# shanice-l/UNOPose

Measured on AMD Instinct MI355X. Metric: (query,ref) pairs/sec forward, higher is better.
Workload: dtype bf16; 1 GPU; UNOPose.forward, batch 32 pairs/GPU, 2048 query pts, 5000->2048 reference pts, 196 coarse pts, 518x518 crops, DINOv2 ViT-B/14 reg4, random-init (trained-like) weights

## Files before the change

### unopose_amd/csrc/gemm_kernel.h

```cpp
#pragma once
#include "gemm_common.h"

namespace unopose {

constexpr int GEMM_XPOL = 2;
#define GEMM_BK 64
constexpr int GEMM_ROTX = 5, GEMM_ROTS = 3;

#define GEMM_WAIT_VM(n) asm volatile("s_waitcnt vmcnt(" #n ")" ::: "memory")
#define GEMM_WAIT_VM_(n) GEMM_WAIT_VM(n)

#define GEMM_LDS_BIAS (2 * GEMM_BUFBYTES)
#define GEMM_LDS_MBOX (GEMM_LDS_BIAS + 2048)
#define GEMM_LDS_LNW (GEMM_LDS_MBOX + 16)
#define GEMM_LDS_LNB (GEMM_LDS_LNW + 1024)
#define GEMM_LDS_LNPART (GEMM_LDS_LNB + 1024)
#define GEMM_LDS_STATS GEMM_LDS_LNPART
#define GEMM_LNF_MAXPARTS 4
#define GEMM_LDS_SHIFT (GEMM_LDS_LNPART + 8192)

template <int EPI, bool GATHER = false, bool F32 = false>
__global__ __launch_bounds__(512, 1) __attribute__((amdgpu_num_vgpr(127))) void gemm256_kernel(const void *__restrict__ Av, const void *__restrict__ Wv,
                                                           const float *__restrict__ bias, void *__restrict__ Cv, int M,
                                                           int N, int K, int tiles_n, int tiles_arg, int nt_store,
                                                           const int *__restrict__ row_list = nullptr,
                                                           const int *__restrict__ tile_info = nullptr,
                                                           const u16 *__restrict__ resid = nullptr, const float *__restrict__ ln_w = nullptr,
                                                           const float *__restrict__ ln_b = nullptr, float ln_eps = 0.f, int lda = 0,
                                                           int ldw = 0, int ldc = 0, int *__restrict__ sched = nullptr,
                                                           void *__restrict__ C2v = nullptr, const float *__restrict__ aux_vec = nullptr,
                                                           float2 *__restrict__ stats = nullptr, int nparts = 0, int stagger = 0,
                                                           const float *__restrict__ fold_prev = nullptr) {
  static_assert(!(F32 && (EPI == 3 || GATHER)), "the fp32-class form has no LayerNorm epilogue / gathered rows");
  static_assert(!((F32 || GATHER) && EPI >= 5), "the residual / LayerNorm-fold epilogues belong to the dense bf16 form");
  constexpr bool LNF = EPI == 6 || EPI == 7;
  static_assert(F32 || EPI != 4, "EPI 4 (bf16 + residual out of fp32-class operands) is an F32 epilogue");
  constexpr int ESZ = F32 ? 4 : 2;
  constexpr int KT = F32 ? 32 : 64;
  const char *A = reinterpret_cast<const char *>(Av), *W = reinterpret_cast<const char *>(Wv);
  const int LDA = lda ? lda : K, LDW = ldw ? ldw : K, LDC = ldc ? ldc : N;
  const int tiles = GATHER ? __builtin_amdgcn_readfirstlane(tile_info[0]) : tiles_arg;
  __shared__ __attribute__((aligned(1024))) char smem[GEMM_LDS_BIAS + 2048 + 16 + (EPI == 3 ? 2048 + 8192 : EPI == 5 ? 2048 + 8192 + 4096 : LNF ? 2048 + 2 * 8192 : 0)];
  float *const lnw_lds = reinterpret_cast<float *>(smem + GEMM_LDS_LNW), *const lnb_lds = reinterpret_cast<float *>(smem + GEMM_LDS_LNB);
  float2 *const ln_part = reinterpret_cast<float2 *>(smem + GEMM_LDS_LNPART);
  if (EPI == 3 && threadIdx.x < GEMM_BN) {
    lnw_lds[threadIdx.x] = ln_w[threadIdx.x];
    lnb_lds[threadIdx.x] = ln_b[threadIdx.x];
  }
  const int tid = threadIdx.x, lane = tid & 63, wave = __builtin_amdgcn_readfirstlane(tid >> 6);
  const int wm = wave >> 2, wn = wave & 3;
  const int l31 = lane & 31, hi = lane >> 5;
  const int l31_ = l31, hi_ = hi, lane_ = lane;
  const int xcd = blockIdx.x & 7, slot = blockIdx.x >> 3, nslots = gridDim.x >> 3;
  const int tiles_m = tiles / tiles_n, per_group = GEMM_GM * tiles_n;
  int cw = (size_t)N * K * ESZ > (size_t)(4u << 20) ? (2400 * 1024) / (GEMM_BN * K * ESZ) : 0;
  if (cw < 3) cw = 0;
  const bool colwalk = cw > 0 && !GATHER && tiles_n > cw && ((tiles_m & 7) == 0 || tiles_m >= 512);
  const int rq = tiles_m >> 3, rr = tiles_m & 7;
  const int rows_x = rq + (xcd < rr ? 1 : 0), row_base = xcd < rr ? xcd * (rq + 1) : rr * (rq + 1) + (xcd - rr) * rq;
  const int cq = tiles >> 3, cr = tiles & 7;
  const int chunk_base = xcd < cr ? xcd * (cq + 1) : cr * (cq + 1) + (xcd - cr) * cq;
  const int chunk_len = colwalk ? rows_x * tiles_n : cq + (xcd < cr ? 1 : 0);
  const __amdgpu_buffer_rsrc_t a_rs = __builtin_amdgcn_make_buffer_rsrc((void *)A, 0, (int)((size_t)M * LDA * ESZ), 0x00020000);
  const __amdgpu_buffer_rsrc_t w_rs = __builtin_amdgcn_make_buffer_rsrc((void *)W, 0, (int)((size_t)N * LDW * ESZ), 0x00020000);
  const __amdgpu_buffer_rsrc_t c_rs = __builtin_amdgcn_make_buffer_rsrc(Cv, 0, GATHER ? 0x7fffffff : (int)((size_t)M * LDC * 2), 0x00020000);
  const __amdgpu_buffer_rsrc_t b_rs = __builtin_amdgcn_make_buffer_rsrc((void *)bias, 0, N * 4, 0x00020000);
  const int nk = K / KT;

  const int fx = (l31 >> 1) & 7;
  uint32_t fr_off[4];
#pragma unroll
  for (int ks = 0; ks < 4; ++ks) fr_off[ks] = (uint32_t)((l31 >> 3) * 1024 + (l31 & 7) * 128 + ((((ks << 1) | hi) ^ fx) << 4));
  const uint32_t a_base = (uint32_t)(wm * 16384);
  const uint32_t w_base = (uint32_t)(GEMM_OPBYTES + wn * 8192);
  const uint32_t a_dst = (uint32_t)((wave >> 2) * 16384 + (wave & 3) * 2048);
  const uint32_t w_dst = (uint32_t)(GEMM_OPBYTES + (wave >> 1) * 8192 + (wave & 1) * 2048);

  struct TileP {
    int m0, n0, rot;
    uint32_t a_off[4], w_off[2];
  };
  auto tile_params = [&](int ti, int step, TileP &p) {
    const int t = chunk_base + ti;
    int tn, tm;
    if (GATHER) {
      tm = t;
      tn = 0;
      const int ng = N / GEMM_BN;
      for (int g = 1; g < ng; ++g) tn += t >= tile_info[1 + g] ? 1 : 0;
      tn = __builtin_amdgcn_readfirstlane(tn);
    } else if (colwalk) {
      const int per_block = rows_x * cw;
      const int cb = ti / per_block, v = ti - cb * per_block;
      const int cwb = min(cw, tiles_n - cb * cw);
      const int g = v / (GEMM_GM * cwb), w = v - g * GEMM_GM * cwb;
      const int gm = min(GEMM_GM, rows_x - g * GEMM_GM);
      const int tl = w / gm;
      tn = cb * cw + tl;
      tm = row_base + g * GEMM_GM + (w - tl * gm);
    } else {
      const int mg = t / per_group, rr = t - mg * per_group;
      const int gm = min(GEMM_GM, tiles_m - mg * GEMM_GM);
      tn = rr / gm;
      tm = mg * GEMM_GM + (rr - tn * gm);
    }
// ... 70 lines not shown
    __syncthreads();
    ti = __builtin_amdgcn_readfirstlane(mbox[0]);
  }
  if (EPI == 5 && stagger > 0 && ((slot / tiles_n) & 1)) {
    const uint64_t t0 = __builtin_amdgcn_s_memrealtime();
    while ((int64_t)(__builtin_amdgcn_s_memrealtime() - t0) < (int64_t)stagger) __builtin_amdgcn_s_sleep(8);
  }
  for (; ti < chunk_len;) {
    const int step = dyn ? ti / nslots : (ti - slot) / nslots;
    if (!have) {
      tile_params(ti, step, cur);
      stage_bias(cur, bsel);
      stage_half(cur, H_A0, 0, par);
      stage_half(cur, H_B0, 0, par);
      stage_half(cur, H_B1, 0, par);
      stage_half(cur, H_A1, 0, par);
      if (nk >= 2) {
        stage_half(cur, H_A0, 1, par ^ GEMM_BUFBYTES);
        stage_half(cur, H_B0, 1, par ^ GEMM_BUFBYTES);
        GEMM_WAIT_VM(6);
      } else {
        GEMM_WAIT_VM(2);
      }
      asm volatile("s_waitcnt lgkmcnt(0)" ::: "memory");
      __builtin_amdgcn_s_barrier();
    }
    const int m0 = __builtin_amdgcn_readfirstlane(cur.m0), n0 = __builtin_amdgcn_readfirstlane(cur.n0);
    cur.rot = __builtin_amdgcn_readfirstlane(cur.rot);
    bool more = can_stream && ti + nslots < chunk_len;
    int ti_next = ti + nslots;
    TileP nxt;

    const float *bias_lds = reinterpret_cast<const float *>(smem + GEMM_LDS_BIAS + bsel * 1024);
    f32x16 acc[2][4];
#pragma unroll
    for (int nb = 0; nb < 2; ++nb)
#pragma unroll
      for (int g = 0; g < 4; ++g) {
        const float4 bv = EPI == 3 || LNF ? make_float4(0.f, 0.f, 0.f, 0.f) : *reinterpret_cast<const float4 *>(bias_lds + wn * 64 + nb * 32 + 8 * g + 4 * hi);
#pragma unroll
        for (int mb = 0; mb < 4; ++mb) {
          acc[nb][mb][4 * g + 0] = bv.x;
          acc[nb][mb][4 * g + 1] = bv.y;
          acc[nb][mb][4 * g + 2] = bv.z;
          acc[nb][mb][4 * g + 3] = bv.w;
        }
      }

    bf16x8 af[2][4], wf0[4], wf1[4];
    auto read_a = [&](const char *lb, int ah) {
#pragma unroll
      for (int mbl = 0; mbl < 2; ++mbl)
#pragma unroll
        for (int ks = 0; ks < 4; ++ks) af[mbl][ks] = *reinterpret_cast<const bf16x8 *>(lb + a_base + ah * 8192 + mbl * 4096 + fr_off[ks]);
    };
    auto read_b = [&](const char *lb, int bh, bf16x8(&wf)[4]) {
#pragma unroll
      for (int ks = 0; ks < 4; ++ks) wf[ks] = *reinterpret_cast<const bf16x8 *>(lb + w_base + bh * 4096 + fr_off[ks]);
    };
    auto mfma_q = [&](int ah, int bh, const bf16x8(&wf)[4]) {
      if (F32) {
#pragma unroll
        for (int b = 0; b < 2; ++b)
#pragma unroll
          for (int mbl = 0; mbl < 2; ++mbl) {
            f32x16 &a = acc[bh][2 * ah + mbl];
            a = __builtin_amdgcn_mfma_f32_32x32x16_bf16(wf[2 + b], af[mbl][b], a, 0, 0, 0);
            a = __builtin_amdgcn_mfma_f32_32x32x16_bf16(wf[b], af[mbl][2 + b], a, 0, 0, 0);
            a = __builtin_amdgcn_mfma_f32_32x32x16_bf16(wf[b], af[mbl][b], a, 0, 0, 0);
          }
        return;
      }
#pragma unroll
      for (int ks = 0; ks < 4; ++ks)
#pragma unroll
        for (int mbl = 0; mbl < 2; ++mbl)
          acc[bh][2 * ah + mbl] = __builtin_amdgcn_mfma_f32_32x32x16_bf16(wf[ks], af[mbl][ks], acc[bh][2 * ah + mbl], 0, 0, 0);
    };
    if (wm == 1) __builtin_amdgcn_s_barrier();
    auto phase = [&](auto compute) {
      asm volatile("s_waitcnt lgkmcnt(0)" ::: "memory");
      __builtin_amdgcn_sched_barrier(0);
      __builtin_amdgcn_s_barrier();
      __builtin_amdgcn_sched_barrier(0);
      compute();
      __builtin_amdgcn_sched_barrier(0);
      __builtin_amdgcn_s_barrier();
      asm volatile("" ::: "memory");
      __builtin_amdgcn_sched_barrier(0);
    };
    for (int t = 0; t < nk; ++t) {
      const bool last = t + 1 == nk, last2 = t + 2 >= nk;
      if (dyn) {
        if (t == 2 && wave == 0) {
          int tk;
          asm volatile("v_readfirstlane_b32 %0, v255" : "=s"(tk)::"memory");
          if (lane == 0) mbox[0] = tk;
        }
        if (t + 2 == nk) {
          ti_next = __builtin_amdgcn_readfirstlane(*reinterpret_cast<volatile int *>(mbox));
          more = ti_next < chunk_len;
        }
      }
      if (more && t + 2 == nk) tile_params(ti_next, dyn ? ti_next / nslots : step + 1, nxt);
      const char *lb = smem + par;
      const uint32_t bnext = par ^ GEMM_BUFBYTES;
      read_b(lb, 0, wf0);
      read_b(lb, 1, wf1);
      read_a(lb, 0);
      __builtin_amdgcn_sched_barrier(0);
// ... 28 lines not shown
        stage_half(cur, H_B0, t + 2, par);
        stage_half(cur, H_B1, t + 2, par);
        GEMM_WAIT_VM(8);
      } else if (more) {
        if (!last) {
          stage_bias(nxt, bsel ^ 1);
          stage_half(nxt, H_A0, 0, par);
          stage_half(nxt, H_B0, 0, par);
          stage_half(nxt, H_B1, 0, par);
          if (LNF) {
            if (nparts <= 3) GEMM_WAIT_VM(9);
            else GEMM_WAIT_VM(10);
          } else
            GEMM_WAIT_VM(8);
        } else if (F32) {
          GEMM_WAIT_VM(2);
        } else {
          stage_half(nxt, H_A0, 1, par);
          stage_half(nxt, H_B0, 1, par);
          GEMM_WAIT_VM(6);
        }
      } else if (!last) {
        GEMM_WAIT_VM(2);
      }
      phase([&] {
        mfma_q(1, 1, wf1);
        mfma_q(1, 0, wf0);
      });
      par ^= GEMM_BUFBYTES;
    }
    if (wm == 0) __builtin_amdgcn_s_barrier();
    par ^= GEMM_BUFBYTES;
    if (EPI == 3) {
#pragma unroll
      for (int mb = 0; mb < 4; ++mb) {
        const int m = min(m0 + wm * 128 + mb * 32 + l31, M - 1);
        const u16 *rp = resid + (size_t)m * GEMM_BN + wn * 64 + 4 * hi;
        float a1 = 0.f, a2 = 0.f;
#pragma unroll
        for (int nb = 0; nb < 2; ++nb)
#pragma unroll
          for (int g = 0; g < 4; ++g) {
            const int nl = nb * 32 + 8 * g + 4 * hi;
            const float4 bv = *reinterpret_cast<const float4 *>(bias_lds + wn * 64 + nl);
            const uint2 r = *reinterpret_cast<const uint2 *>(rp + nb * 32 + 8 * g);
            const float v0 = acc[nb][mb][4 * g + 0] + bv.x + __uint_as_float(r.x << 16);
            const float v1 = acc[nb][mb][4 * g + 1] + bv.y + __uint_as_float(r.x & 0xffff0000u);
            const float v2 = acc[nb][mb][4 * g + 2] + bv.z + __uint_as_float(r.y << 16);
            const float v3 = acc[nb][mb][4 * g + 3] + bv.w + __uint_as_float(r.y & 0xffff0000u);
            acc[nb][mb][4 * g + 0] = v0;
            acc[nb][mb][4 * g + 1] = v1;
            acc[nb][mb][4 * g + 2] = v2;
            acc[nb][mb][4 * g + 3] = v3;
            a1 += (v0 + v1) + (v2 + v3);
            a2 += (v0 * v0 + v1 * v1) + (v2 * v2 + v3 * v3);
          }
        a1 += __shfl_xor(a1, 32);
        a2 += __shfl_xor(a2, 32);
        if (hi == 0) ln_part[((wm * 4 + mb) * 32 + l31) * 4 + wn] = make_float2(a1, a2);
      }
      __syncthreads();
#pragma unroll
      for (int mb = 0; mb < 4; ++mb) {
        const float2 *pp = ln_part + ((wm * 4 + mb) * 32 + l31) * 4;
        const float t1 = (pp[0].x + pp[1].x) + (pp[2].x + pp[3].x), t2 = (pp[0].y + pp[1].y) + (pp[2].y + pp[3].y);
        const float mean = t1 * (1.f / GEMM_BN);
        const float rstd = rsqrtf(fmaxf(t2 * (1.f / GEMM_BN) - mean * mean, 0.f) + ln_eps);
#pragma unroll
        for (int nb = 0; nb < 2; ++nb)
#pragma unroll
          for (int g = 0; g < 4; ++g) {
            const int nl = wn * 64 + nb * 32 + 8 * g + 4 * hi;
            const float4 gw = *reinterpret_cast<const float4 *>(lnw_lds + nl), gb = *reinterpret_cast<const float4 *>(lnb_lds + nl);
            acc[nb][mb][4 * g + 0] = (acc[nb][mb][4 * g + 0] - mean) * rstd * gw.x + gb.x;
            acc[nb][mb][4 * g + 1] = (acc[nb][mb][4 * g + 1] - mean) * rstd * gw.y + gb.y;
            acc[nb][mb][4 * g + 2] = (acc[nb][mb][4 * g + 2] - mean) * rstd * gw.z + gb.z;
            acc[nb][mb][4 * g + 3] = (acc[nb][mb][4 * g + 3] - mean) * rstd * gw.w + gb.w;
          }
      }
    }
    if constexpr (LNF) {
      int l31 = l31_, hi = hi_;
      asm volatile("" : "+v"(l31), "+v"(hi));
      const float *c_lds = reinterpret_cast<const float *>(smem + GEMM_LDS_LNW + bsel * 1024);
      const float inv_k = 1.f / (float)K;
      float rs[4], nm[4];
#pragma unroll
      for (int mb = 0; mb < 4; ++mb) {
        const float2 *sp = reinterpret_cast<const float2 *>(smem + GEMM_LDS_STATS + bsel * 8192) + (wm * 128 + mb * 32 + l31) * nparts;
        float t1 = 0.f, t2 = 0.f;
#pragma unroll
        for (int i = 0; i < GEMM_LNF_MAXPARTS; ++i)
          if (i < nparts) {
            const float2 q = sp[i];
            t1 += q.x;
            t2 += q.y;
          }
        const float mean = t1 * inv_k;
        rs[mb] = rsqrtf(fmaxf(t2 * inv_k - mean * mean, 0.f) + ln_eps);
        nm[mb] = -mean * rs[mb];
      }
#pragma unroll
      for (int nb = 0; nb < 2; ++nb)
#pragma unroll
        for (int g = 0; g < 4; ++g) {
          const int nl = wn * 64 + nb * 32 + 8 * g + 4 * hi;
          const float4 cv = *reinterpret_cast<const float4 *>(c_lds + nl), dv = *reinterpret_cast<const float4 *>(bias_lds + nl);
#pragma unroll
          for (int mb = 0; mb < 4; ++mb) {
            acc[nb][mb][4 * g + 0] = fmaf(rs[mb], acc[nb][mb][4 * g + 0], fmaf(nm[mb], cv.x, dv.x));
            acc[nb][mb][4 * g + 1] = fmaf(rs[mb], acc[nb][mb][4 * g + 1], fmaf(nm[mb], cv.y, dv.y));
            acc[nb][mb][4 * g + 2] = fmaf(rs[mb], acc[nb][mb][4 * g + 2], fmaf(nm[mb], cv.z, dv.z));
            acc[nb][mb][4 * g + 3] = fmaf(rs[mb], acc[nb][mb][4 * g + 3], fmaf(nm[mb], cv.w, dv.w));
          }
        }
    }
    if constexpr (EPI == 5) {
      int l31 = l31_, hi = hi_, lane = lane_;
      asm volatile("" : "+v"(l31), "+v"(hi), "+v"(lane));
      char *cw = smem + par + (wave < 4 ? 8192 + (wave & 1) * 4096 + (wave >> 1) * 16384 : GEMM_OPBYTES + 4096 + (wave - 4) * 8192);
      const __amdgpu_buffer_rsrc_t x_rs = __builtin_amdgcn_make_buffer_rsrc(C2v, 0, (int)((size_t)M * N * 4), 0x00020000);
      const int r4 = lane >> 4, q = lane & 15;
      const uint32_t x_v0 = (uint32_t)((((size_t)m0 + wm * 128 + r4) * N + n0 + wn * 64 + q * 4) * 4);
      const uint32_t c_v0 = (uint32_t)((((size_t)m0 + wm * 128 + r4) * LDC + n0 + wn * 64 + q * 4) * 2);
      const uint32_t x_rowb = (uint32_t)(N * 4), c_rowb = (uint32_t)(LDC * 2);
      const int rows_p = tiles_m * GEMM_BM;
      float sv[2] = {0.f, 0.f};
      if (fold_prev != nullptr) {
        float pv[2][GEMM_LNF_MAXPARTS + 1];
#pragma unroll
        for (int j = 0; j < 2; ++j) {
          const size_t m = (size_t)m0 + wm * 128 + j * 64 + lane, sh_at = (size_t)rows_p * 2 * nparts + m;
#pragma unroll
          for (int i = 0; i < GEMM_LNF_MAXPARTS; ++i) pv[j][i] = fold_prev[i < nparts ? m * 2 * nparts + 2 * i : sh_at];
          pv[j][GEMM_LNF_MAXPARTS] = fold_prev[sh_at];
        }
#pragma unroll
        for (int j = 0; j < 2; ++j) {
          float t = 0.f;
#pragma unroll
          for (int i = 0; i < GEMM_LNF_MAXPARTS; ++i) t += i < nparts ? pv[j][i] : 0.f;
          sv[j] = m0 + wm * 128 + j * 64 + lane < M ? pv[j][GEMM_LNF_MAXPARTS] + t * (1.f / (float)N) : 0.f;
        }
      }
      constexpr int PF = 3;
      f32x4 rv[PF][4];
      auto load_round = [&](int r, f32x4(&dst)[4]) {
#pragma unroll
        for (int it = 0; it < 4; ++it) {
          dst[it] = __builtin_bit_cast(f32x4, __builtin_amdgcn_raw_buffer_load_b128(x_rs, x_v0 + (uint32_t)(r * 16 + it * 4) * x_rowb, 0, GEMM_XPOL));
        }
      };
#pragma unroll
      for (int r = 0; r < PF; ++r) load_round(r, rv[r]);
      float *const sh_lds = reinterpret_cast<float *>(smem + GEMM_LDS_SHIFT + wave * 512);
#pragma unroll
      for (int r = 0; r < 8; ++r) {
        const int mb = r >> 1, h = r & 1;
        if ((l31 >> 4) == h) {
#pragma unroll
          for (int nb = 0; nb < 2; ++nb)
#pragma unroll
            for (int g = 0; g < 4; ++g) {
              const int s16 = (nb * 8 + 2 * g + hi) ^ (l31 & 15);
              *reinterpret_cast<float4 *>(cw + (l31 & 15) * 256 + s16 * 16) =
                  make_float4(acc[nb][mb][4 * g + 0], acc[nb][mb][4 * g + 1], acc[nb][mb][4 * g + 2], acc[nb][mb][4 * g + 3]);
            }
        }
        if (r == 0) {
#pragma unroll
          for (int j = 0; j < 2; ++j) {
            sh_lds[j * 64 + lane] = sv[j];
            if (wn == 0) reinterpret_cast<float *>(stats)[(size_t)rows_p * 2 * tiles_n + m0 + wm * 128 + j * 64 + lane] = sv[j];
          }
        }
        __builtin_amdgcn_fence(__ATOMIC_RELEASE, "wavefront");
        __builtin_amdgcn_wave_barrier();
        __builtin_amdgcn_fence(__ATOMIC_ACQUIRE, "wavefront");
#pragma unroll
        for (int it = 0; it < 4; ++it) {
          const int row = it * 4 + r4;
          const f32x4 a = *reinterpret_cast<const f32x4 *>(cw + row * 256 + ((q ^ row) << 4));
          const f32x4 o = rv[r % PF][it];
          f32x4 v;
#pragma unroll
          for (int e = 0; e < 4; ++e) v[e] = a[e] + o[e];
          __builtin_amdgcn_raw_buffer_store_b128(__builtin_bit_cast(u32x4, v), x_rs, x_v0 + (uint32_t)(r * 16 + it * 4) * x_rowb, 0, GEMM_XPOL);
          const float s = sh_lds[row + r * 16];
#pragma unroll
          for (int e = 0; e < 4; ++e) v[e] = v[e] - s;
          typedef unsigned int u32x2 __attribute__((ext_vector_type(2)));
          const u32x2 pk = {cvt_pk_bf16_f32(v[0], v[1]), cvt_pk_bf16_f32(v[2], v[3])};
          if (nt_store)
            __builtin_amdgcn_raw_buffer_store_b64(pk, c_rs, c_v0 + (uint32_t)(r * 16 + it * 4) * c_rowb, 0, 2);
          else
            __builtin_amdgcn_raw_buffer_store_b64(pk, c_rs, c_v0 + (uint32_t)(r * 16 + it * 4) * c_rowb, 0, 0);
          float a1 = (v[0] + v[1]) + (v[2] + v[3]), a2 = (v[0] * v[0] + v[1] * v[1]) + (v[2] * v[2] + v[3] * v[3]);
          a1 += dpp_f32<0x111, 0xF>(a1, 0.f);
          a2 += dpp_f32<0x111, 0xF>(a2, 0.f);
          a1 += dpp_f32<0x112, 0xF>(a1, 0.f);
          a2 += dpp_f32<0x112, 0xF>(a2, 0.f);
          a1 += dpp_f32<0x114, 0xF>(a1, 0.f);
          a2 += dpp_f32<0x114, 0xF>(a2, 0.f);
          a1 += dpp_f32<0x118, 0xF>(a1, 0.f);
          a2 += dpp_f32<0x118, 0xF>(a2, 0.f);
          if (q == 15) ln_part[((wm * 4 + mb) * 32 + h * 16 + row) * 4 + wn] = make_float2(a1, a2);
        }
        __builtin_amdgcn_fence(__ATOMIC_RELEASE, "wavefront");
        __builtin_amdgcn_wave_barrier();
        __builtin_amdgcn_fence(__ATOMIC_ACQUIRE, "wavefront");
        if (r + PF < 8) load_round(r + PF, rv[r % PF]);
      }
      asm volatile("s_waitcnt lgkmcnt(0)" ::: "memory");
      __builtin_amdgcn_s_barrier();
      if (wn == 0 && hi == 0) {
#pragma unroll
        for (int mb = 0; mb < 4; ++mb) {
          const float2 *pp = ln_part + ((wm * 4 + mb) * 32 + l31) * 4;
          const float4 p01 = *reinterpret_cast<const float4 *>(pp), p23 = *reinterpret_cast<const float4 *>(pp + 2);
          stats[(size_t)(m0 + wm * 128 + mb * 32 + l31) * tiles_n + (n0 >> 8)] = make_float2((p01.x + p01.z) + (p23.x + p23.z), (p01.y + p01.w) + (p23.y + p23.w));
        }
      }
    } else if constexpr (!F32) {
    int l31 = l31_, hi = hi_, lane = lane_;
    asm volatile("" : "+v"(l31), "+v"(hi), "+v"(lane));
    char *cw = smem + par + (wave < 4 ? 8192 + (wave & 1) * 4096 + (wave >> 1) * 16384 : GEMM_OPBYTES + 4096 + (wave - 4) * 8192);
    const uint32_t c_v0 = GATHER ? (uint32_t)((((size_t)m0 + wm * 128 + (lane >> 3)) * GEMM_BN + wn * 64 + (lane & 7) * 8) * 2)
                                 : (uint32_t)((((size_t)m0 + wm * 128 + (lane >> 3)) * LDC + n0 + wn * 64 + (lane & 7) * 8) * 2);
    const uint32_t c_rowb = (uint32_t)((GATHER ? GEMM_BN : LDC) * 2);
#pragma unroll
    for (int mb = 0; mb < 4; ++mb) {
#pragma unroll
      for (int nb = 0; nb < 2; ++nb) {
#pragma unroll
        for (int g = 0; g < 4; ++g) {
          const int nl = nb * 32 + 8 * g + 4 * hi;
          float v0 = acc[nb][mb][4 * g + 0], v1 = acc[nb][mb][4 * g + 1], v2 = acc[nb][mb][4 * g + 2], v3 = acc[nb][mb][4 * g + 3];
          if (EPI == 1 || EPI == 7) {
            v0 = gelu_bf16_class(v0);
            v1 = gelu_bf16_class(v1);
            v2 = gelu_bf16_class(v2);
            v3 = gelu_bf16_class(v3);
          }
          if (EPI == 2) {
            v0 = fmaxf(v0, 0.f);
            v1 = fmaxf(v1, 0.f);
            v2 = fmaxf(v2, 0.f);
            v3 = fmaxf(v3, 0.f);
          }
          const int slot16 = (nl >> 3) ^ (l31 & 7);
          *reinterpret_cast<uint2 *>(cw + l31 * 128 + slot16 * 16 + (nl & 4) * 2) = make_uint2(cvt_pk_bf16_f32(v0, v1), cvt_pk_bf16_f32(v2, v3));
        }
      }
      __builtin_amdgcn_fence(__ATOMIC_RELEASE, "wavefront");
      __builtin_amdgcn_wave_barrier();
      __builtin_amdgcn_fence(__ATOMIC_ACQUIRE, "wavefront");
      u32x4 cv[4];
#pragma unroll
      for (int it = 0; it < 4; ++it) {
        const int row = it * 8 + (lane >> 3), q = lane & 7;
        cv[it] = *reinterpret_cast<const u32x4 *>(cw + row * 128 + ((q ^ (row & 7)) << 4));
      }
#pragma unroll
      for (int it = 0; it < 4; ++it) {
        const uint32_t off = c_v0 + (uint32_t)(mb * 32 + it * 8) * c_rowb;
        if (nt_store)
          __builtin_amdgcn_raw_buffer_store_b128(cv[it], c_rs, off, 0, 2);
        else
          __builtin_amdgcn_raw_buffer_store_b128(cv[it], c_rs, off, 0, 0);
      }
      __builtin_amdgcn_fence(__ATOMIC_RELEASE, "wavefront");
      __builtin_amdgcn_wave_barrier();
      __builtin_amdgcn_fence(__ATOMIC_ACQUIRE, "wavefront");
    }
    } else {
    int l31 = l31_, hi = hi_, lane = lane_;
    asm volatile("" : "+v"(l31), "+v"(hi), "+v"(lane));
    char *cw = smem + par + wave * 8192;
    const __amdgpu_buffer_rsrc_t cf_rs = __builtin_amdgcn_make_buffer_rsrc(Cv, 0, (int)((size_t)M * N * (EPI == 4 ? 2 : 4)), 0x00020000);
    const __amdgpu_buffer_rsrc_t cs_rs = __builtin_amdgcn_make_buffer_rsrc(C2v, 0, (int)((size_t)M * N * 4), 0x00020000);
    const __amdgpu_buffer_rsrc_t rs_rs = __builtin_amdgcn_make_buffer_rsrc((void *)resid, 0, (int)((size_t)M * N * 2), 0x00020000);
    const bool has_cf = Cv != nullptr, has_cs = C2v != nullptr;
    const uint32_t c32_v0 = (uint32_t)((((size_t)m0 + wm * 128 + (lane >> 4)) * N + n0 + wn * 64 + (lane & 15) * 4) * 4);
    const uint32_t c16_v0 = (uint32_t)((((size_t)m0 + wm * 128 + (lane >> 3)) * N + n0 + wn * 64 + (lane & 7) * 8) * 2);
#pragma unroll
    for (int mb = 0; mb < 4; ++mb) {
      auto vals = [&](int nb, int g, float (&x)[4]) {
#pragma unroll
        for (int e = 0; e < 4; ++e) {
          float t = acc[nb][mb][4 * g + e];
          if (EPI == 1) t = gelu_erf(t);
          if (EPI == 2) t = fmaxf(t, 0.f);
          x[e] = t;
        }
        __builtin_amdgcn_sched_barrier(0);
      };
      if (EPI == 4) {
#pragma unroll
        for (int nb = 0; nb < 2; ++nb)
#pragma unroll
          for (int g = 0; g < 4; ++g) {
            float x[4];
            vals(nb, g, x);
            *reinterpret_cast<uint2 *>(cw + l31 * 128 + (((nb * 4 + g) ^ (l31 & 7)) << 4) + hi * 8) =
                make_uint2(cvt_pk_bf16_f32(x[0], x[1]), cvt_pk_bf16_f32(x[2], x[3]));
          }
        __builtin_amdgcn_fence(__ATOMIC_RELEASE, "wavefront");
        __builtin_amdgcn_wave_barrier();
        __builtin_amdgcn_fence(__ATOMIC_ACQUIRE, "wavefront");
#pragma unroll
        for (int it = 0; it < 4; ++it) {
          const int row = it * 8 + (lane >> 3), q = lane & 7;
          u32x4 o = *reinterpret_cast<const u32x4 *>(cw + row * 128 + ((q ^ (row & 7)) << 4));
          const uint32_t off = c16_v0 + (uint32_t)(mb * 32 + it * 8) * (uint32_t)(N * 2);
          if (resid) {
            const u32x4 r = __builtin_amdgcn_raw_buffer_load_b128(rs_rs, off, 0, 0);
#pragma unroll
            for (int e = 0; e < 4; ++e)
              o[e] = cvt_pk_bf16_f32(__uint_as_float(o[e] << 16) + __uint_as_float(r[e] << 16),
                                     __uint_as_float(o[e] & 0xffff0000u) + __uint_as_float(r[e] & 0xffff0000u));
          }
          __builtin_amdgcn_raw_buffer_store_b128(o, cf_rs, off, 0, 0);
        }
        __builtin_amdgcn_fence(__ATOMIC_RELEASE, "wavefront");
        __builtin_amdgcn_wave_barrier();
        __builtin_amdgcn_fence(__ATOMIC_ACQUIRE, "wavefront");
        continue;
      }
      if (has_cf) {
#pragma unroll
        for (int nb = 0; nb < 2; ++nb)
#pragma unroll
          for (int g = 0; g < 4; ++g) {
            float x[4];
            vals(nb, g, x);
            const int s = (nb * 8 + 2 * g + hi) ^ (l31 & 15);
            *reinterpret_cast<float4 *>(cw + l31 * 256 + s * 16) = make_float4(x[0], x[1], x[2], x[3]);
          }
        __builtin_amdgcn_fence(__ATOMIC_RELEASE, "wavefront");
        __builtin_amdgcn_wave_barrier();
        __builtin_amdgcn_fence(__ATOMIC_ACQUIRE, "wavefront");
#pragma unroll
        for (int it = 0; it < 8; ++it) {
          const int row = it * 4 + (lane >> 4), q = lane & 15;
          const u32x4 o = *reinterpret_cast<const u32x4 *>(cw + row * 256 + ((q ^ (row & 15)) << 4));
          const uint32_t off = c32_v0 + (uint32_t)(mb * 32 + it * 4) * (uint32_t)(N * 4);
          if (nt_store)
            __builtin_amdgcn_raw_buffer_store_b128(o, cf_rs, off, 0, 2);
          else
            __builtin_amdgcn_raw_buffer_store_b128(o, cf_rs, off, 0, 0);
        }
        __builtin_amdgcn_fence(__ATOMIC_RELEASE, "wavefront");
        __builtin_amdgcn_wave_barrier();
        __builtin_amdgcn_fence(__ATOMIC_ACQUIRE, "wavefront");
      }
      if (has_cs) {
#pragma unroll
        for (int nb = 0; nb < 2; ++nb)
#pragma unroll
          for (int g = 0; g < 4; ++g) {
            float x[4];
            vals(nb, g, x);
            const uint32_t h0 = cvt_pk_bf16_f32(x[0], x[1]), h1 = cvt_pk_bf16_f32(x[2], x[3]);
            const float r0 = x[0] - __uint_as_float(h0 << 16), r1 = x[1] - __uint_as_float(h0 & 0xffff0000u);
            const float r2 = x[2] - __uint_as_float(h1 << 16), r3 = x[3] - __uint_as_float(h1 & 0xffff0000u);
            const uint32_t l0 = cvt_pk_bf16_f32(r0, r1), l1 = cvt_pk_bf16_f32(r2, r3);
            const int sh = (nb * 8 + g) ^ (l31 & 15), sl = (nb * 8 + 4 + g) ^ (l31 & 15);
            *reinterpret_cast<uint2 *>(cw + l31 * 256 + sh * 16 + hi * 8) = make_uint2(h0, h1);
            *reinterpret_cast<uint2 *>(cw + l31 * 256 + sl * 16 + hi * 8) = make_uint2(l0, l1);
          }
        __builtin_amdgcn_fence(__ATOMIC_RELEASE, "wavefront");
        __builtin_amdgcn_wave_barrier();
        __builtin_amdgcn_fence(__ATOMIC_ACQUIRE, "wavefront");
#pragma unroll
        for (int it = 0; it < 8; ++it) {
          const int row = it * 4 + (lane >> 4), q = lane & 15;
          const u32x4 o = *reinterpret_cast<const u32x4 *>(cw + row * 256 + ((q ^ (row & 15)) << 4));
          __builtin_amdgcn_raw_buffer_store_b128(o, cs_rs, c32_v0 + (uint32_t)(mb * 32 + it * 4) * (uint32_t)(N * 4), 0, 0);
        }
        __builtin_amdgcn_fence(__ATOMIC_RELEASE, "wavefront");
        __builtin_amdgcn_wave_barrier();
        __builtin_amdgcn_fence(__ATOMIC_ACQUIRE, "wavefront");
      }
    }
    }
    par ^= GEMM_BUFBYTES;
    asm volatile("s_waitcnt lgkmcnt(0)" ::: "memory");
    __builtin_amdgcn_s_barrier();
    if (F32 && more) {
      stage_half(nxt, H_A0, 1, par ^ GEMM_BUFBYTES);
      stage_half(nxt, H_B0, 1, par ^ GEMM_BUFBYTES);
    }
    have = more;
    if (more) {
      cur = nxt;
      bsel ^= 1;
    }
    ti = ti_next;
  }
  if (dyn && tid == 0) {
    if (atomicAdd(sched + 8, 1) == (int)gridDim.x - 1) {
#pragma unroll
// ... 7 lines not shown
```

Baseline: 1101 pairs/s.

## Switch GEMM accumulators from 32x32x16 to 16x16x32 MFMA tiles via AccTile abstraction

Replaces the 32x32x16 bf16 MFMA accumulator layout with 16x16x32 MFMA fragments, behind an AccTile helper that defines row/part mapping, fragment LDS offsets and column groups. All epilogues (LayerNorm, LN-fold, residual, bf16 and fp32 stores) are remapped to the new lane-to-element layout. The fp32-class GELU is also hoisted into one pass over the accumulators. This aims for better MFMA issue and LDS read patterns, at the cost of more instructions per tile and a risk of register pressure or layout bugs under the 127 VGPR cap.

Result: faster. 1127 pairs/s (median of 6 runs) (+2.3%).

```diff
diff --git a/unopose_amd/csrc/gemm_kernel.h b/unopose_amd/csrc/gemm_kernel.h
--- a/unopose_amd/csrc/gemm_kernel.h
+++ b/unopose_amd/csrc/gemm_kernel.h
@@ -18,6 +18,25 @@
 #define GEMM_LDS_STATS GEMM_LDS_LNPART
 #define GEMM_LNF_MAXPARTS 4
 #define GEMM_LDS_SHIFT (GEMM_LDS_LNPART + 8192)
+
+struct AccTile {
+  static constexpr int RB = 16;
+  static constexpr int NRB = 128 / RB;
+  static constexpr int NP = 64 / RB;
+  static constexpr int NCG = 16 / NP;
+  static constexpr int NKS = 8 / NP;
+  typedef f32x4 frag;
+  static __device__ __forceinline__ int row(int lane) { return lane & (RB - 1); }
+  static __device__ __forceinline__ int part(int lane) { return (lane / RB) & (NP - 1); }
+  static __device__ __forceinline__ int col0(int cg, int pt) { return cg * (4 * NP) + 4 * pt; }
+  static __device__ __forceinline__ f32x4 get(const frag (&acc)[NCG][NRB], int rb, int cg) { return acc[cg][rb]; }
+  static __device__ __forceinline__ void set(frag (&acc)[NCG][NRB], int rb, int cg, f32x4 v) { acc[cg][rb] = v; }
+  static __device__ __forceinline__ uint32_t frag_off(int ks, int lane) {
+    const int r = row(lane), c = NP * ks + part(lane);
+    return (uint32_t)((r >> 3) * 1024 + (r & 7) * 128 + ((c ^ ((r >> 1) & 7)) << 4));
+  }
+  static __device__ __forceinline__ frag mfma(bf16x8 w, bf16x8 a, frag c) { return __builtin_amdgcn_mfma_f32_16x16x32_bf16(w, a, c, 0, 0, 0); }
+};
 
 template <int EPI, bool GATHER = false, bool F32 = false>
 __global__ __launch_bounds__(512, 1) __attribute__((amdgpu_num_vgpr(127))) void gemm256_kernel(const void *__restrict__ Av, const void *__restrict__ Wv,
@@ -37,6 +56,8 @@
   static_assert(F32 || EPI != 4, "EPI 4 (bf16 + residual out of fp32-class operands) is an F32 epilogue");
   constexpr int ESZ = F32 ? 4 : 2;
   constexpr int KT = F32 ? 32 : 64;
+  using T = AccTile;
+  using frag = T::frag;
   const char *A = reinterpret_cast<const char *>(Av), *W = reinterpret_cast<const char *>(Wv);
   const int LDA = lda ? lda : K, LDW = ldw ? ldw : K, LDC = ldc ? ldc : N;
   const int tiles = GATHER ? __builtin_amdgcn_readfirstlane(tile_info[0]) : tiles_arg;
@@ -49,8 +70,7 @@
   }
   const int tid = threadIdx.x, lane = tid & 63, wave = __builtin_amdgcn_readfirstlane(tid >> 6);
   const int wm = wave >> 2, wn = wave & 3;
-  const int l31 = lane & 31, hi = lane >> 5;
-  const int l31_ = l31, hi_ = hi, lane_ = lane;
+  const int lane_ = lane;
   const int xcd = blockIdx.x & 7, slot = blockIdx.x >> 3, nslots = gridDim.x >> 3;
   const int tiles_m = tiles / tiles_n, per_group = GEMM_GM * tiles_n;
   int cw = (size_t)N * K * ESZ > (size_t)(4u << 20) ? (2400 * 1024) / (GEMM_BN * K * ESZ) : 0;
@@ -67,10 +87,10 @@
   const __amdgpu_buffer_rsrc_t b_rs = __builtin_amdgcn_make_buffer_rsrc((void *)bias, 0, N * 4, 0x00020000);
   const int nk = K / KT;
 
-  const int fx = (l31 >> 1) & 7;
-  uint32_t fr_off[4];
-#pragma unroll
-  for (int ks = 0; ks < 4; ++ks) fr_off[ks] = (uint32_t)((l31 >> 3) * 1024 + (l31 & 7) * 128 + ((((ks << 1) | hi) ^ fx) << 4));
+  uint32_t fr_off[T::NKS];
+#pragma unroll
+  for (int ks = 0; ks < T::NKS; ++ks) fr_off[ks] = T::frag_off(ks, lane);
+  constexpr int ABH = 64 / T::RB, BBH = 32 / T::RB, BLKB = T::RB * GEMM_ROWB;
   const uint32_t a_base = (uint32_t)(wm * 16384);
   const uint32_t w_base = (uint32_t)(GEMM_OPBYTES + wn * 8192);
   const uint32_t a_dst = (uint32_t)((wave >> 2) * 16384 + (wave & 3) * 2048);
@@ -207,50 +227,54 @@
     TileP nxt;
 
     const float *bias_lds = reinterpret_cast<const float *>(smem + GEMM_LDS_BIAS + bsel * 1024);
-    f32x16 acc[2][4];
-#pragma unroll
-    for (int nb = 0; nb < 2; ++nb)
-#pragma unroll
-      for (int g = 0; g < 4; ++g) {
-        const float4 bv = EPI == 3 || LNF ? make_float4(0.f, 0.f, 0.f, 0.f) : *reinterpret_cast<const float4 *>(bias_lds + wn * 64 + nb * 32 + 8 * g + 4 * hi);
-#pragma unroll
-        for (int mb = 0; mb < 4; ++mb) {
-          acc[nb][mb][4 * g + 0] = bv.x;
-          acc[nb][mb][4 * g + 1] = bv.y;
-          acc[nb][mb][4 * g + 2] = bv.z;
-          acc[nb][mb][4 * g + 3] = bv.w;
-        }
-      }
-
-    bf16x8 af[2][4], wf0[4], wf1[4];
+    frag acc[T::NCG][T::NRB];
+    {
+      const int pt = T::part(lane);
+#pragma unroll
+      for (int cg = 0; cg < T::NCG; ++cg) {
+        const float4 bv = EPI == 3 || LNF ? make_float4(0.f, 0.f, 0.f, 0.f) : *reinterpret_cast<const float4 *>(bias_lds + wn * 64 + T::col0(cg, pt));
+#pragma unroll
+        for (int rb = 0; rb < T::NRB; ++rb) T::set(acc, rb, cg, f32x4{bv.x, bv.y, bv.z, bv.w});
+      }
+    }
+
+    bf16x8 af[ABH * T::NKS], wf0[BBH * T::NKS], wf1[BBH * T::NKS];
     auto read_a = [&](const char *lb, int ah) {
 #pragma unroll
-      for (int mbl = 0; mbl < 2; ++mbl)
-#pragma unroll
-        for (int ks = 0; ks < 4; ++ks) af[mbl][ks] = *reinterpret_cast<const bf16x8 *>(lb + a_base + ah * 8192 + mbl * 4096 + fr_off[ks]);
+      for (int mbl = 0; mbl < ABH; ++mbl)
+#pragma unroll
+        for (int ks = 0; ks < T::NKS; ++ks)
+          af[mbl * T::NKS + ks] = *reinterpret_cast<const bf16x8 *>(lb + a_base + ah * 8192 + mbl * BLKB + fr_off[ks]);
     };
-    auto read_b = [&](const char *lb, int bh, bf16x8(&wf)[4]) {
-#pragma unroll
-      for (int ks = 0; ks < 4; ++ks) wf[ks] = *reinterpret_cast<const bf16x8 *>(lb + w_base + bh * 4096 + fr_off[ks]);
+    auto read_b = [&](const char *lb, int bh, bf16x8(&wf)[BBH * T::NKS]) {
+#pragma unroll
+      for (int nbl = 0; nbl < BBH; ++nbl)
+#pragma unroll
+        for (int ks = 0; ks < T::NKS; ++ks)
+          wf[nbl * T::NKS + ks] = *reinterpret_cast<const bf16x8 *>(lb + w_base + bh * 4096 + nbl * BLKB + fr_off[ks]);
     };
-    auto mfma_q = [&](int ah, int bh, const bf16x8(&wf)[4]) {
-      if (F32) {
-#pragma unroll
-        for (int b = 0; b < 2; ++b)
-#pragma unroll
-          for (int mbl = 0; mbl < 2; ++mbl) {
-            f32x16 &a = acc[bh][2 * ah + mbl];
-            a = __builtin_amdgcn_mfma_f32_32x32x16_bf16(wf[2 + b], af[mbl][b], a, 0, 0, 0);
-            a = __builtin_amdgcn_mfma_f32_32x32x16_bf16(wf[b], af[mbl][2 + b], a, 0, 0, 0);
-            a = __builtin_amdgcn_mfma_f32_32x32x16_bf16(wf[b], af[mbl][b], a, 0, 0, 0);
-          }
-        return;
-      }
-#pragma unroll
-      for (int ks = 0; ks < 4; ++ks)
-#pragma unroll
-        for (int mbl = 0; mbl < 2; ++mbl)
-          acc[bh][2 * ah + mbl] = __builtin_amdgcn_mfma_f32_32x32x16_bf16(wf[ks], af[mbl][ks], acc[bh][2 * ah + mbl], 0, 0, 0);
+    auto mfma_q = [&](int ah, int bh, const bf16x8(&wf)[BBH * T::NKS]) {
+      if constexpr (F32) {
+#pragma unroll
+        for (int term = 0; term < 3; ++term)
+#pragma unroll
+          for (int nbl = 0; nbl < BBH; ++nbl)
+#pragma unroll
+            for (int mbl = 0; mbl < ABH; ++mbl) {
+              frag &a = acc[bh * BBH + nbl][ah * ABH + mbl];
+              a = T::mfma(wf[nbl * T::NKS + (term == 0 ? 1 : 0)], af[mbl * T::NKS + (term == 1 ? 1 : 0)], a);
+            }
+      } else {
+#pragma unroll
+        for (int ks = 0; ks < T::NKS; ++ks)
+#pragma unroll
+          for (int nbl = 0; nbl < BBH; ++nbl)
+#pragma unroll
+            for (int mbl = 0; mbl < ABH; ++mbl) {
+              frag &a = acc[bh * BBH + nbl][ah * ABH + mbl];
+              a = T::mfma(wf[nbl * T::NKS + ks], af[mbl * T::NKS + ks], a);
+            }
+      }
     };
     if (wm == 1) __builtin_amdgcn_s_barrier();
     auto phase = [&](auto compute) {
@@ -345,62 +369,61 @@
     if (wm == 0) __builtin_amdgcn_s_barrier();
     par ^= GEMM_BUFBYTES;
     if (EPI == 3) {
-#pragma unroll
-      for (int mb = 0; mb < 4; ++mb) {
-        const int m = min(m0 + wm * 128 + mb * 32 + l31, M - 1);
-        const u16 *rp = resid + (size_t)m * GEMM_BN + wn * 64 + 4 * hi;
+      const int row = T::row(lane), pt = T::part(lane);
+#pragma unroll
+      for (int rb = 0; rb < T::NRB; ++rb) {
+        const int m = min(m0 + wm * 128 + rb * T::RB + row, M - 1);
+        const u16 *rp = resid + (size_t)m * GEMM_BN + wn * 64;
         float a1 = 0.f, a2 = 0.f;
 #pragma unroll
-        for (int nb = 0; nb < 2; ++nb)
-#pragma unroll
-          for (int g = 0; g < 4; ++g) {
-            const int nl = nb * 32 + 8 * g + 4 * hi;
-            const float4 bv = *reinterpret_cast<const float4 *>(bias_lds + wn * 64 + nl);
-            const uint2 r = *reinterpret_cast<const uint2 *>(rp + nb * 32 + 8 * g);
-            const float v0 = acc[nb][mb][4 * g + 0] + bv.x + __uint_as_float(r.x << 16);
-            const float v1 = acc[nb][mb][4 * g + 1] + bv.y + __uint_as_float(r.x & 0xffff0000u);
-            const float v2 = acc[nb][mb][4 * g + 2] + bv.z + __uint_as_float(r.y << 16);
-            const float v3 = acc[nb][mb][4 * g + 3] + bv.w + __uint_as_float(r.y & 0xffff0000u);
-            acc[nb][mb][4 * g + 0] = v0;
-            acc[nb][mb][4 * g + 1] = v1;
-            acc[nb][mb][4 * g + 2] = v2;
-            acc[nb][mb][4 * g + 3] = v3;
-            a1 += (v0 + v1) + (v2 + v3);
-            a2 += (v0 * v0 + v1 * v1) + (v2 * v2 + v3 * v3);
-          }
-        a1 += __shfl_xor(a1, 32);
-        a2 += __shfl_xor(a2, 32);
-        if (hi == 0) ln_part[((wm * 4 + mb) * 32 + l31) * 4 + wn] = make_float2(a1, a2);
+        for (int cg = 0; cg < T::NCG; ++cg) {
+          const int nl = T::col0(cg, pt);
+          const f32x4 bv = *reinterpret_cast<const f32x4 *>(bias_lds + wn * 64 + nl);
+          const uint2 r = *reinterpret_cast<const uint2 *>(rp + nl);
+          f32x4 v = T::get(acc, rb, cg);
+          v[0] = v[0] + bv[0] + __uint_as_float(r.x << 16);
+          v[1] = v[1] + bv[1] + __uint_as_float(r.x & 0xffff0000u);
+          v[2] = v[2] + bv[2] + __uint_as_float(r.y << 16);
+          v[3] = v[3] + bv[3] + __uint_as_float(r.y & 0xffff0000u);
+          T::set(acc, rb, cg, v);
+          a1 += (v[0] + v[1]) + (v[2] + v[3]);
+          a2 += (v[0] * v[0] + v[1] * v[1]) + (v[2] * v[2] + v[3] * v[3]);
+        }
+#pragma unroll
+        for (int d = T::RB; d < 64; d <<= 1) {
+          a1 += __shfl_xor(a1, d);
+          a2 += __shfl_xor(a2, d);
+        }
+        if (pt == 0) ln_part[(wm * 128 + rb * T::RB + row) * 4 + wn] = make_float2(a1, a2);
       }
       __syncthreads();
 #pragma unroll
-      for (int mb = 0; mb < 4; ++mb) {
-        const float2 *pp = ln_part + ((wm * 4 + mb) * 32 + l31) * 4;
+      for (int rb = 0; rb < T::NRB; ++rb) {
+        const float2 *pp = ln_part + (wm * 128 + rb * T::RB + row) * 4;
         const float t1 = (pp[0].x + pp[1].x) + (pp[2].x + pp[3].x), t2 = (pp[0].y + pp[1].y) + (pp[2].y + pp[3].y);
         const float mean = t1 * (1.f / GEMM_BN);
         const float rstd = rsqrtf(fmaxf(t2 * (1.f / GEMM_BN) - mean * mean, 0.f) + ln_eps);
 #pragma unroll
-        for (int nb = 0; nb < 2; ++nb)
-#pragma unroll
-          for (int g = 0; g < 4; ++g) {
-            const int nl = wn * 64 + nb * 32 + 8 * g + 4 * hi;
-            const float4 gw = *reinterpret_cast<const float4 *>(lnw_lds + nl), gb = *reinterpret_cast<const float4 *>(lnb_lds + nl);
-            acc[nb][mb][4 * g + 0] = (acc[nb][mb][4 * g + 0] - mean) * rstd * gw.x + gb.x;
-            acc[nb][mb][4 * g + 1] = (acc[nb][mb][4 * g + 1] - mean) * rstd * gw.y + gb.y;
-            acc[nb][mb][4 * g + 2] = (acc[nb][mb][4 * g + 2] - mean) * rstd * gw.z + gb.z;
-            acc[nb][mb][4 * g + 3] = (acc[nb][mb][4 * g + 3] - mean) * rstd * gw.w + gb.w;
-          }
+        for (int cg = 0; cg < T::NCG; ++cg) {
+          const int nl = wn * 64 + T::col0(cg, pt);
+          const f32x4 gw = *reinterpret_cast<const f32x4 *>(lnw_lds + nl), gb = *reinterpret_cast<const f32x4 *>(lnb_lds + nl);
+          f32x4 v = T::get(acc, rb, cg);
+#pragma unroll
+          for (int e = 0; e < 4; ++e) v[e] = (v[e] - mean) * rstd * gw[e] + gb[e];
+          T::set(acc, rb, cg, v);
+        }
       }
     }
     if constexpr (LNF) {
-      int l31 = l31_, hi = hi_;
-      asm volatile("" : "+v"(l31), "+v"(hi));
+      int lane = lane_;
+      asm volatile("" : "+v"(lane));
+      const int row = T::row(lane), pt = T::part(lane);
       const float *c_lds = reinterpret_cast<const float *>(smem + GEMM_LDS_LNW + bsel * 1024);
       const float inv_k = 1.f / (float)K;
-      float rs[4], nm[4];
-#pragma unroll
-      for (int mb = 0; mb < 4; ++mb) {
-        const float2 *sp = reinterpret_cast<const float2 *>(smem + GEMM_LDS_STATS + bsel * 8192) + (wm * 128 + mb * 32 + l31) * nparts;
+      float rs[T::NRB], nm[T::NRB];
+#pragma unroll
+      for (int rb = 0; rb < T::NRB; ++rb) {
+        const float2 *sp = reinterpret_cast<const float2 *>(smem + GEMM_LDS_STATS + bsel * 8192) + (wm * 128 + rb * T::RB + row) * nparts;
         float t1 = 0.f, t2 = 0.f;
 #pragma unroll
         for (int i = 0; i < GEMM_LNF_MAXPARTS; ++i)
@@ -410,27 +433,26 @@
             t2 += q.y;
           }
         const float mean = t1 * inv_k;
-        rs[mb] = rsqrtf(fmaxf(t2 * inv_k - mean * mean, 0.f) + ln_eps);
-        nm[mb] = -mean * rs[mb];
-      }
-#pragma unroll
-      for (int nb = 0; nb < 2; ++nb)
-#pragma unroll
-        for (int g = 0; g < 4; ++g) {
-          const int nl = wn * 64 + nb * 32 + 8 * g + 4 * hi;
-          const float4 cv = *reinterpret_cast<const float4 *>(c_lds + nl), dv = *reinterpret_cast<const float4 *>(bias_lds + nl);
-#pragma unroll
-          for (int mb = 0; mb < 4; ++mb) {
-            acc[nb][mb][4 * g + 0] = fmaf(rs[mb], acc[nb][mb][4 * g + 0], fmaf(nm[mb], cv.x, dv.x));
-            acc[nb][mb][4 * g + 1] = fmaf(rs[mb], acc[nb][mb][4 * g + 1], fmaf(nm[mb], cv.y, dv.y));
-            acc[nb][mb][4 * g + 2] = fmaf(rs[mb], acc[nb][mb][4 * g + 2], fmaf(nm[mb], cv.z, dv.z));
-            acc[nb][mb][4 * g + 3] = fmaf(rs[mb], acc[nb][mb][4 * g + 3], fmaf(nm[mb], cv.w, dv.w));
-          }
-        }
+        rs[rb] = rsqrtf(fmaxf(t2 * inv_k - mean * mean, 0.f) + ln_eps);
+        nm[rb] = -mean * rs[rb];
+      }
+#pragma unroll
+      for (int cg = 0; cg < T::NCG; ++cg) {
+        const int nl = wn * 64 + T::col0(cg, pt);
+        const f32x4 cv = *reinterpret_cast<const f32x4 *>(c_lds + nl), dv = *reinterpret_cast<const f32x4 *>(bias_lds + nl);
+#pragma unroll
+        for (int rb = 0; rb < T::NRB; ++rb) {
+          f32x4 v = T::get(acc, rb, cg);
+#pragma unroll
+          for (int e = 0; e < 4; ++e) v[e] = fmaf(rs[rb], v[e], fmaf(nm[rb], cv[e], dv[e]));
+          T::set(acc, rb, cg, v);
+        }
+      }
     }
     if constexpr (EPI == 5) {
-      int l31 = l31_, hi = hi_, lane = lane_;
-      asm volatile("" : "+v"(l31), "+v"(hi), "+v"(lane));
+      int lane = lane_;
+      asm volatile("" : "+v"(lane));
+      const int arow = T::row(lane), pt = T::part(lane);
       char *cw = smem + par + (wave < 4 ? 8192 + (wave & 1) * 4096 + (wave >> 1) * 16384 : GEMM_OPBYTES + 4096 + (wave - 4) * 8192);
       const __amdgpu_buffer_rsrc_t x_rs = __builtin_amdgcn_make_buffer_rsrc(C2v, 0, (int)((size_t)M * N * 4), 0x00020000);
       const int r4 = lane >> 4, q = lane & 15;
@@ -469,16 +491,11 @@
       float *const sh_lds = reinterpret_cast<float *>(smem + GEMM_LDS_SHIFT + wave * 512);
 #pragma unroll
       for (int r = 0; r < 8; ++r) {
-        const int mb = r >> 1, h = r & 1;
-        if ((l31 >> 4) == h) {
-#pragma unroll
-          for (int nb = 0; nb < 2; ++nb)
-#pragma unroll
-            for (int g = 0; g < 4; ++g) {
-              const int s16 = (nb * 8 + 2 * g + hi) ^ (l31 & 15);
-              *reinterpret_cast<float4 *>(cw + (l31 & 15) * 256 + s16 * 16) =
-                  make_float4(acc[nb][mb][4 * g + 0], acc[nb][mb][4 * g + 1], acc[nb][mb][4 * g + 2], acc[nb][mb][4 * g + 3]);
-            }
+        static_assert(T::RB == 16, "a staging round of the residual epilogue is one row block");
+#pragma unroll
+        for (int cg = 0; cg < T::NCG; ++cg) {
+          const int s16 = (T::col0(cg, pt) >> 2) ^ arow;
+          *reinterpret_cast<f32x4 *>(cw + arow * 256 + s16 * 16) = T::get(acc, r, cg);
         }
         if (r == 0) {
 #pragma unroll
@@ -517,7 +534,7 @@
           a2 += dpp_f32<0x114, 0xF>(a2, 0.f);
           a1 += dpp_f32<0x118, 0xF>(a1, 0.f);
           a2 += dpp_f32<0x118, 0xF>(a2, 0.f);
-          if (q == 15) ln_part[((wm * 4 + mb) * 32 + h * 16 + row) * 4 + wn] = make_float2(a1, a2);
+          if (q == 15) ln_part[(wm * 128 + r * 16 + row) * 4 + wn] = make_float2(a1, a2);
         }
         __builtin_amdgcn_fence(__ATOMIC_RELEASE, "wavefront");
         __builtin_amdgcn_wave_barrier();
@@ -526,17 +543,18 @@
       }
       asm volatile("s_waitcnt lgkmcnt(0)" ::: "memory");
       __builtin_amdgcn_s_barrier();
-      if (wn == 0 && hi == 0) {
+      if (wn == 0 && lane < 32) {
 #pragma unroll
         for (int mb = 0; mb < 4; ++mb) {
-          const float2 *pp = ln_part + ((wm * 4 + mb) * 32 + l31) * 4;
+          const float2 *pp = ln_part + (wm * 128 + mb * 32 + lane) * 4;
           const float4 p01 = *reinterpret_cast<const float4 *>(pp), p23 = *reinterpret_cast<const float4 *>(pp + 2);
-          stats[(size_t)(m0 + wm * 128 + mb * 32 + l31) * tiles_n + (n0 >> 8)] = make_float2((p01.x + p01.z) + (p23.x + p23.z), (p01.y + p01.w) + (p23.y + p23.w));
+          stats[(size_t)(m0 + wm * 128 + mb * 32 + lane) * tiles_n + (n0 >> 8)] = make_float2((p01.x + p01.z) + (p23.x + p23.z), (p01.y + p01.w) + (p23.y + p23.w));
         }
       }
     } else if constexpr (!F32) {
-    int l31 = l31_, hi = hi_, lane = lane_;
-    asm volatile("" : "+v"(l31), "+v"(hi), "+v"(lane));
+    int lane = lane_;
+    asm volatile("" : "+v"(lane));
+    const int arow = T::row(lane), pt = T::part(lane);
     char *cw = smem + par + (wave < 4 ? 8192 + (wave & 1) * 4096 + (wave >> 1) * 16384 : GEMM_OPBYTES + 4096 + (wave - 4) * 8192);
     const uint32_t c_v0 = GATHER ? (uint32_t)((((size_t)m0 + wm * 128 + (lane >> 3)) * GEMM_BN + wn * 64 + (lane & 7) * 8) * 2)
                                  : (uint32_t)((((size_t)m0 + wm * 128 + (lane >> 3)) * LDC + n0 + wn * 64 + (lane & 7) * 8) * 2);
@@ -544,11 +562,13 @@
 #pragma unroll
     for (int mb = 0; mb < 4; ++mb) {
 #pragma unroll
-      for (int nb = 0; nb < 2; ++nb) {
-#pragma unroll
-        for (int g = 0; g < 4; ++g) {
-          const int nl = nb * 32 + 8 * g + 4 * hi;
-          float v0 = acc[nb][mb][4 * g + 0], v1 = acc[nb][mb][4 * g + 1], v2 = acc[nb][mb][4 * g + 2], v3 = acc[nb][mb][4 * g + 3];
+      for (int j = 0; j < 32 / T::RB; ++j) {
+        const int rl = j * T::RB + arow;
+#pragma unroll
+        for (int cg = 0; cg < T::NCG; ++cg) {
+          const int nl = T::col0(cg, pt);
+          const f32x4 av = T::get(acc, mb * (32 / T::RB) + j, cg);
+          float v0 = av[0], v1 = av[1], v2 = av[2], v3 = av[3];
           if (EPI == 1 || EPI == 7) {
             v0 = gelu_bf16_class(v0);
             v1 = gelu_bf16_class(v1);
@@ -561,8 +581,8 @@
             v2 = fmaxf(v2, 0.f);
             v3 = fmaxf(v3, 0.f);
           }
-          const int slot16 = (nl >> 3) ^ (l31 & 7);
-          *reinterpret_cast<uint2 *>(cw + l31 * 128 + slot16 * 16 + (nl & 4) * 2) = make_uint2(cvt_pk_bf16_f32(v0, v1), cvt_pk_bf16_f32(v2, v3));
+          const int slot16 = (nl >> 3) ^ (rl & 7);
+          *reinterpret_cast<uint2 *>(cw + rl * 128 + slot16 * 16 + (nl & 4) * 2) = make_uint2(cvt_pk_bf16_f32(v0, v1), cvt_pk_bf16_f32(v2, v3));
         }
       }
       __builtin_amdgcn_fence(__ATOMIC_RELEASE, "wavefront");
@@ -587,8 +607,10 @@
       __builtin_amdgcn_fence(__ATOMIC_ACQUIRE, "wavefront");
     }
     } else {
-    int l31 = l31_, hi = hi_, lane = lane_;
-    asm volatile("" : "+v"(l31), "+v"(hi), "+v"(lane));
+    int lane = lane_;
+    asm volatile("" : "+v"(lane));
+    const int arow = T::row(lane), pt = T::part(lane);
+    constexpr int JB = 32 / T::RB;
     char *cw = smem + par + wave * 8192;
     const __amdgpu_buffer_rsrc_t cf_rs = __builtin_amdgcn_make_buffer_rsrc(Cv, 0, (int)((size_t)M * N * (EPI == 4 ? 2 : 4)), 0x00020000);
     const __amdgpu_buffer_rsrc_t cs_rs = __builtin_amdgcn_make_buffer_rsrc(C2v, 0, (int)((size_t)M * N * 4), 0x00020000);
@@ -596,13 +618,24 @@
     const bool has_cf = Cv != nullptr, has_cs = C2v != nullptr;
     const uint32_t c32_v0 = (uint32_t)((((size_t)m0 + wm * 128 + (lane >> 4)) * N + n0 + wn * 64 + (lane & 15) * 4) * 4);
     const uint32_t c16_v0 = (uint32_t)((((size_t)m0 + wm * 128 + (lane >> 3)) * N + n0 + wn * 64 + (lane & 7) * 8) * 2);
+    if (EPI == 1) {
+#pragma unroll
+      for (int rb = 0; rb < T::NRB; ++rb)
+#pragma unroll
+        for (int cg = 0; cg < T::NCG; ++cg) {
+          f32x4 v = T::get(acc, rb, cg);
+#pragma unroll
+          for (int e = 0; e < 4; ++e) v[e] = gelu_erf(v[e]);
+          T::set(acc, rb, cg, v);
+          __builtin_amdgcn_sched_barrier(0);
+        }
+    }
 #pragma unroll
     for (int mb = 0; mb < 4; ++mb) {
-      auto vals = [&](int nb, int g, float (&x)[4]) {
+      auto vals = [&](int j, int cg, float (&x)[4]) {
 #pragma unroll
         for (int e = 0; e < 4; ++e) {
-          float t = acc[nb][mb][4 * g + e];
-          if (EPI == 1) t = gelu_erf(t);
+          float t = T::get(acc, mb * JB + j, cg)[e];
           if (EPI == 2) t = fmaxf(t, 0.f);
           x[e] = t;
         }
@@ -610,12 +643,13 @@
       };
       if (EPI == 4) {
 #pragma unroll
-        for (int nb = 0; nb < 2; ++nb)
-#pragma unroll
-          for (int g = 0; g < 4; ++g) {
+        for (int j = 0; j < JB; ++j)
+#pragma unroll
+          for (int cg = 0; cg < T::NCG; ++cg) {
             float x[4];
-            vals(nb, g, x);
-            *reinterpret_cast<uint2 *>(cw + l31 * 128 + (((nb * 4 + g) ^ (l31 & 7)) << 4) + hi * 8) =
+            vals(j, cg, x);
+            const int rl = j * T::RB + arow, nl = T::col0(cg, pt);
+            *reinterpret_cast<uint2 *>(cw + rl * 128 + (((nl >> 3) ^ (rl & 7)) << 4) + (nl & 4) * 2) =
                 make_uint2(cvt_pk_bf16_f32(x[0], x[1]), cvt_pk_bf16_f32(x[2], x[3]));
           }
         __builtin_amdgcn_fence(__ATOMIC_RELEASE, "wavefront");
@@ -642,13 +676,13 @@
       }
       if (has_cf) {
 #pragma unroll
-        for (int nb = 0; nb < 2; ++nb)
-#pragma unroll
-          for (int g = 0; g < 4; ++g) {
+        for (int j = 0; j < JB; ++j)
+#pragma unroll
+          for (int cg = 0; cg < T::NCG; ++cg) {
             float x[4];
-            vals(nb, g, x);
-            const int s = (nb * 8 + 2 * g + hi) ^ (l31 & 15);
-            *reinterpret_cast<float4 *>(cw + l31 * 256 + s * 16) = make_float4(x[0], x[1], x[2], x[3]);
+            vals(j, cg, x);
+            const int rl = j * T::RB + arow, s = (T::col0(cg, pt) >> 2) ^ (rl & 15);
+            *reinterpret_cast<float4 *>(cw + rl * 256 + s * 16) = make_float4(x[0], x[1], x[2], x[3]);
           }
         __builtin_amdgcn_fence(__ATOMIC_RELEASE, "wavefront");
         __builtin_amdgcn_wave_barrier();
@@ -669,18 +703,20 @@
       }
       if (has_cs) {
 #pragma unroll
-        for (int nb = 0; nb < 2; ++nb)
-#pragma unroll
-          for (int g = 0; g < 4; ++g) {
+        for (int j = 0; j < JB; ++j)
+#pragma unroll
+          for (int cg = 0; cg < T::NCG; ++cg) {
             float x[4];
-            vals(nb, g, x);
+            vals(j, cg, x);
+            const int rl = j * T::RB + arow, nl = T::col0(cg, pt);
             const uint32_t h0 = cvt_pk_bf16_f32(x[0], x[1]), h1 = cvt_pk_bf16_f32(x[2], x[3]);
             const float r0 = x[0] - __uint_as_float(h0 << 16), r1 = x[1] - __uint_as_float(h0 & 0xffff0000u);
             const float r2 = x[2] - __uint_as_float(h1 << 16), r3 = x[3] - __uint_as_float(h1 & 0xffff0000u);
             const uint32_t l0 = cvt_pk_bf16_f32(r0, r1), l1 = cvt_pk_bf16_f32(r2, r3);
-            const int sh = (nb * 8 + g) ^ (l31 & 15), sl = (nb * 8 + 4 + g) ^ (l31 & 15);
-            *reinterpret_cast<uint2 *>(cw + l31 * 256 + sh * 16 + hi * 8) = make_uint2(h0, h1);
-            *reinterpret_cast<uint2 *>(cw + l31 * 256 + sl * 16 + hi * 8) = make_uint2(l0, l1);
+            const int s0 = (nl >> 5) * 8 + ((nl & 31) >> 3);
+            const int sh = s0 ^ (rl & 15), sl = (s0 + 4) ^ (rl & 15);
+            *reinterpret_cast<uint2 *>(cw + rl * 256 + sh * 16 + (nl & 4) * 2) = make_uint2(h0, h1);
+            *reinterpret_cast<uint2 *>(cw + rl * 256 + sl * 16 + (nl & 4) * 2) = make_uint2(l0, l1);
           }
         __builtin_amdgcn_fence(__ATOMIC_RELEASE, "wavefront");
         __builtin_amdgcn_wave_barrier();
```
